# youtalk/opencv-ar

Hardware: AMD Instinct MI355X
Metric: frames/sec at 1920x1080, 16 markers/frame; 1/2/4/8 MI355X (higher is better)
Workload: dtype u8

## Files before the change

opencv-ar_amd/csrc/api.hip:

```cpp
#include "context.h"
#include "plan_core.h"
#include <algorithm>
#include <cstdlib>
#include <cstring>
#include <new>

using namespace ocvar;

static_assert(sizeof(TemplateRec) == sizeof(OcvarTemplate) && sizeof(TemplateRec) == 48, "CvarTemplate layout");
static_assert(MAX_SIZE_CLASSES == OCVAR_MAX_TEMPLATE_SIZES, "size classes");
static_assert(sizeof(CameraRec) == sizeof(OcvarCamera) && sizeof(CameraRec) == 248, "CvarCamera layout");
static_assert(sizeof(MarkerRec) == sizeof(OcvarMarker) && sizeof(MarkerRec) == 184, "CvarMarker layout");
static_assert(sizeof(BoardEntry) == sizeof(OcvarBoardMarker) && sizeof(BoardEntry) == 72, "OcvarBoardMarker layout");
static_assert(sizeof(BoardPose) == sizeof(OcvarBoardPose) && sizeof(BoardPose) == 192, "OcvarBoardPose layout");

template <typename T>
static int dev_alloc(OcvarHip* c, T** p, size_t n) {
    void* q = nullptr;
    HIP_TRY(c, hipMalloc(&q, n * sizeof(T) + 256));
    c->allocs.push_back(q);
    *p = static_cast<T*>(q);
    return OCVAR_OK;
}

static int create_impl(OcvarHip** out, int device, int max_width, int max_height, int max_batch, int max_quads, int max_markers,
                       bool dense) {
    if (!out || max_width < 16 || max_height < 16 || max_width > 32767 || max_height > 32767 || max_batch < 1 || max_quads < 1 ||
        max_markers < 1)
        return OCVAR_E_ARG;
    *out = nullptr;
    int ndev = 0;
    if (hipGetDeviceCount(&ndev) != hipSuccess || ndev <= 0 || device < 0 || device >= ndev) return OCVAR_E_NO_DEVICE;
    hipDeviceProp_t prop;
    if (hipGetDeviceProperties(&prop, device) != hipSuccess) return OCVAR_E_NO_DEVICE;
    if (std::strncmp(prop.gcnArchName, "gfx950", 6) != 0) {
        std::fprintf(stderr, "ocvar_hip: device %d is %s; this library carries gfx950 code only\n", device, prop.gcnArchName);
        return OCVAR_E_NO_DEVICE;
    }
    OcvarHip* c = new (std::nothrow) OcvarHip();
    if (!c) return OCVAR_E_HIP;
    *out = c;
    c->device = device;
    HIP_TRY(c, hipSetDevice(device));
    HIP_TRY(c, c->stream.ensure(hipStreamNonBlocking));
    for (auto& e : c->ev) HIP_TRY(c, e.ensure(hipEventDefault));
    Workspace& w = c->ws;
    plan_workspace(&w, max_width, max_height, max_batch, max_quads, max_markers, dense);
    c->result_limit = max_markers;
    const size_t B = (size_t)max_batch, M = (size_t)max_markers;
    int rc;
    if ((rc = dev_alloc(c, &w.gray, B * (size_t)gray_plane_bytes(max_width, max_height)))) return rc;
    if ((rc = dev_alloc(c, &w.nbr_frame, B * (size_t)nbr_plane_bytes(((max_width & ~1) + 15) & ~15, max_height & ~1)))) return rc;
    if ((rc = dev_alloc(c, &w.nbr_crop, (size_t)w.cap_crop_pixels))) return rc;
    if ((rc = dev_alloc(c, &w.cands_frame, (size_t)w.cap_frame_cands))) return rc;
    if ((rc = dev_alloc(c, &w.cands_crop, (size_t)w.cap_crop_cands))) return rc;
    if ((rc = dev_alloc(c, &w.pool, (size_t)w.cap_pool_ints))) return rc;
    if ((rc = dev_alloc(c, &w.slab, (size_t)w.max_mid_blocks * 256 * SLAB_STRIDE))) return rc;
    if ((rc = dev_alloc(c, &w.slab3, (size_t)w.max_long_blocks * 4 * SLAB3_STRIDE))) return rc;
    if ((rc = dev_alloc(c, &w.mid_frame, (size_t)w.cap_long))) return rc;
    if ((rc = dev_alloc(c, &w.mid_crop, (size_t)w.cap_long))) return rc;
    if ((rc = dev_alloc(c, &w.mid_first_crop, (size_t)w.cap_long))) return rc;
    if ((rc = dev_alloc(c, &w.long_frame, (size_t)w.cap_long))) return rc;
    if ((rc = dev_alloc(c, &w.long_crop, (size_t)w.cap_long))) return rc;
    if ((rc = dev_alloc(c, &w.quads_frame, B * max_quads))) return rc;
    if ((rc = dev_alloc(c, &w.n_quads_frame, B))) return rc;
    if ((rc = dev_alloc(c, &w.squares, B * max_quads * 8))) return rc;
    if ((rc = dev_alloc(c, &w.n_squares, B))) return rc;
    if ((rc = dev_alloc(c, &w.crop_of, B * max_quads))) return rc;
    if ((rc = dev_alloc(c, &w.rois_crop, (size_t)w.cap_crop_rois))) return rc;
    if ((rc = dev_alloc(c, &w.tiles_crop, (size_t)w.cap_crop_tiles))) return rc;
    if ((rc = dev_alloc(c, &w.quads_crop, (size_t)w.cap_crop_quads))) return rc;
    if ((rc = dev_alloc(c, &w.best_crop, (size_t)w.cap_crop_rois))) return rc;
    if ((rc = dev_alloc(c, &w.crop_min_rest, (size_t)w.cap_crop_rois))) return rc;
    if ((rc = dev_alloc(c, &w.ring_frame, B))) return rc;
    if ((rc = dev_alloc(c, &w.ring_crop, (size_t)w.cap_crop_rois))) return rc;
    if ((rc = dev_alloc(c, &w.sq_recs, B * max_quads))) return rc;
    if ((rc = dev_alloc(c, &w.prev, B * M))) return rc;
    if ((rc = dev_alloc(c, &w.n_prev, B))) return rc;
    if ((rc = dev_alloc(c, &w.reserve, B * M))) return rc;
    if ((rc = dev_alloc(c, &w.n_reserve, B))) return rc;
    if ((rc = dev_alloc(c, &w.markers, B * M))) return rc;
    if ((rc = dev_alloc(c, &w.pose_jobs, B * M))) return rc;
    if (dense) {
        const int nc = w.track_gw * w.track_gh;
        if ((rc = dev_alloc(c, &w.sorted_starts, B * max_quads))) return rc;
        if ((rc = dev_alloc(c, &w.sq_tmp, B * max_quads * 8))) return rc;
        if ((rc = dev_alloc(c, &w.trk_cells, B * (nc + 1)))) return rc;
        if ((rc = dev_alloc(c, &w.trk_fill, B * nc))) return rc;
        if ((rc = dev_alloc(c, &w.trk_items, B * 4 * max_quads))) return rc;
        if ((rc = dev_alloc(c, &w.trk_next, B * (max_quads + 1)))) return rc;
        if ((rc = dev_alloc(c, &w.surv, B * max_quads))) return rc;
        if ((rc = dev_alloc(c, &w.src, B * M))) return rc;
    }
    if ((rc = dev_alloc(c, &w.n_markers, B))) return rc;
    if ((rc = dev_alloc(c, &w.templates, (size_t)MAXT))) return rc;
    if ((rc = dev_alloc(c, &w.sizes, (size_t)MAX_SIZE_CLASSES))) return rc;
    if ((rc = dev_alloc(c, &w.lut, (size_t)4 * MAXT))) return rc;
    if ((rc = dev_alloc(c, &w.group_off, (size_t)MAXT + 1))) return rc;
    if ((rc = dev_alloc(c, &w.group_members, (size_t)MAXT))) return rc;
    if ((rc = dev_alloc(c, &w.camera, (size_t)1))) return rc;
    if ((rc = dev_alloc(c, &w.counters, (size_t)CNT_COUNT))) return rc;

    w.crop_pixels = reinterpret_cast<unsigned long long*>(w.counters + CNT_CROP_PIXELS);
    HIP_TRY(c, hipMemset(w.n_prev, 0, B * sizeof(int)));
    HIP_TRY(c, hipMemset(w.counters, 0, CNT_COUNT * sizeof(int)));
    HIP_TRY(c, c->h_markers.reserve(B * M * sizeof(MarkerRec)));
    HIP_TRY(c, c->h_counts.reserve(B * sizeof(int)));
    HIP_TRY(c, c->h_prev.reserve(B * M * sizeof(MarkerRec)));
    HIP_TRY(c, c->h_prev_counts.reserve(B * sizeof(int)));
    HIP_TRY(c, c->h_counters.reserve(CNT_COUNT * sizeof(int)));
    return OCVAR_OK;
}

extern "C" int ocvar_hip_create(OcvarHip** out, int device, int max_width, int max_height, int max_batch) {
    return ocvar_hip_create_ex(out, device, max_width, max_height, max_batch, OCVAR_MAX_QUADS);
}

extern "C" int ocvar_hip_create_ex(OcvarHip** out, int device, int max_width, int max_height, int max_batch, int max_quads) {
    if (max_quads < 1 || max_quads > OCVAR_MAX_QUADS_EX) return OCVAR_E_ARG;
    return create_impl(out, device, max_width, max_height, max_batch, max_quads, OCVAR_MAX_MARKERS, false);
}

extern "C" int ocvar_hip_create_dense(OcvarHip** out, int device, int max_width, int max_height, int max_batch, int max_quads,
                                      int max_markers) {
    if (max_quads < 1 || max_quads > OCVAR_MAX_QUADS_DENSE || max_markers < 1 || max_markers > OCVAR_MAX_MARKERS_DENSE) return OCVAR_E_ARG;
    return create_impl(out, device, max_width, max_height, max_batch, max_quads, max_markers, true);
}

extern "C" int ocvar_hip_max_markers(const OcvarHip* c) { return c ? c->ws.maxm : OCVAR_E_ARG; }

OcvarHip::~OcvarHip() {
    for (void* p : allocs) (void)hipFree(p);
    if (!h_overlays) return;
    for (auto& t : h_overlays->tex)
        if (t.px) (void)hipFree(const_cast<uint32_t*>(t.px));
    delete h_overlays;
}

extern "C" void ocvar_hip_destroy(OcvarHip* c) {
    if (!c) return;
    (void)hipSetDevice(c->device);
    gate_detach(c);
    if (c->stream) (void)hipStreamSynchronize(c->stream);
    if (c->ovl_used) (void)hipEventSynchronize(c->ovl_done);
// ... 681 lines not shown
```

opencv-ar_amd/csrc/follow.hip:

```cpp
#include "kernels.h"
#include "trace_core.h"

namespace ocvar {

__device__ __forceinline__ int ticket_lane() {
    int l = (int)(threadIdx.x & 63);
    asm volatile("" : "+v"(l));
    return l;
}
__device__ __forceinline__ int uni(int v) { return __builtin_amdgcn_readfirstlane(v); }
__device__ __forceinline__ unsigned uni(unsigned v) { return (unsigned)__builtin_amdgcn_readfirstlane((int)v); }
__device__ __forceinline__ unsigned long long uni(unsigned long long v) {
    return ((unsigned long long)uni((unsigned)(v >> 32)) << 32) | uni((unsigned)v);
}
__device__ __forceinline__ double uni(double v) { return __longlong_as_double((long long)uni((unsigned long long)__double_as_longlong(v))); }

#ifdef OCVAR_PROF
#define PROF_NOW() __builtin_readcyclecounter()
#define PROF_DECL() unsigned long long prof_acc[16] = {0, 0, 0, 0, 0, 0, 0, 0, 0, 0, 0, 0, 0, 0, 0, 0}
#define PROF_ADD(slot, v) do { prof_acc[slot] += (unsigned long long)(v); } while (0)
#define PROF_FLUSH(base) do { if ((threadIdx.x & 63) == 0) for (int i_ = 0; i_ < 16; i_++) if (i_ != 7) atomicAdd(reinterpret_cast<unsigned long long*>(ws.counters + CNT_PROF) + (base) + i_, prof_acc[i_]); } while (0)
#else
#define PROF_NOW() 0ull
#define PROF_DECL() do { } while (0)
// ... 277 lines not shown
        px = ex;
        py = ey;
    }
    __builtin_amdgcn_fence(__ATOMIC_ACQ_REL, "workgroup");
    return new_count;
}

template <bool CROP, bool STAGE>
__device__ __forceinline__ bool wave_finish_packed(const Workspace& ws, const StartCand c, const PlaneRef& pl, const unsigned* gsrc, int npts,
                                                   unsigned* lpts, WaveScratch* sc) {
    const int lane = threadIdx.x & 63;
    if (npts < 4) return false;
    unsigned lo = 0xffffffffu, hi = 0u;
    if (STAGE) {
        unsigned v[LDS_PTS / 64];
#pragma unroll
        for (int k = 0; k < LDS_PTS / 64; k++) {
            const int i = lane + 64 * k;
            v[k] = i < npts ? gsrc[i] : 0u;
        }
#pragma unroll
        for (int k = 0; k < LDS_PTS / 64; k++) {
            const int i = lane + 64 * k;
            if (i < npts) {
                lpts[i] = v[k];
                lo = pk_min(lo, v[k]);
                hi = pk_max(hi, v[k]);
            }
        }
    } else {
        for (int i = lane; i < npts; i += 64) {
            const unsigned p = gsrc[i];
            lo = pk_min(lo, p);
            hi = pk_max(hi, p);
        }
    }
    lo = wave_pk_min(lo);
    hi = wave_pk_max(hi);
    const int bw = px_of(hi) - px_of(lo), bh = py_of(hi) - py_of(lo);
    if (!((long long)bw * bh > 500)) return false;
    __builtin_amdgcn_fence(__ATOMIC_ACQ_REL, "workgroup");
    const unsigned* src = STAGE ? lpts : gsrc;
    double per = 0.0;
    for (int i = lane; i < npts; i += 64) {
        const unsigned p = src[i], q = src[i == 0 ? npts - 1 : i - 1];
        const float dx = (float)px_of(p) - (float)px_of(q), dy = (float)py_of(p) - (float)py_of(q);
        per += (double)sqrt_rn(dx * dx + dy * dy);
    }
    per = wave_sum_f64(per);
#ifdef OCVAR_PROF
    if (lane == 0) atomicAdd(reinterpret_cast<unsigned long long*>(ws.counters + CNT_PROF) + (CROP ? 16 : 0) + 7, 1ull);
#endif
    const bool k32 = npts <= 1024 && (long long)bw * bw + (long long)bh * bh < (1ll << 21);
    const int m = k32 ? wave_approx_dp<true>(src, npts, per * 0.02, sc->dst, sc->stack) : wave_approx_dp<false>(src, npts, per * 0.02, sc->dst, sc->stack);
    if (m != 4) return false;
    int q[8];
#pragma unroll
    for (int k = 0; k < 8; k++) q[k] = uni(sc->dst[k]);
    if (!quad_filter(q, pl.img_w, pl.img_h)) return false;
    if (lane == 0) emit_quad<CROP>(ws, c, q);
    return true;
}

template <bool CROP>
__device__ __forceinline__ int follow_short(const Workspace& ws, const StartCand c) {
    const int BUDGET = SHORT_STEPS;
    const PlaneRef pl = plane_of<CROP>(ws, c.roi);
    if (c.pos <= 0 || c.pos >= pl.plane) return false;
    {
        if (earlier_start_behind(pl.nbr, pl.ns, pl.plane, c.pos, c.is_hole, BACK_STEPS)) return 0;
        if (CROP) {
            const int x = c.pos % pl.ns, y = c.pos / pl.ns;
            return (x == 1 || y == 1) ? 3 : 1;
        }
        const LeanTrace lt = trace_flat(pl.nbr, pl.ns, pl.plane, c.pos, c.is_hole, nullptr, 0, BUDGET);
        if (lt.status == TRACE_OVERRUN) return lt.npts <= 2 ? 2 : 1;
        if (lt.status != TRACE_OK || lt.npts < 4) return 0;
        return 1;
    }
    return 0;
}

template <bool CROP>
__device__ int follow_overflow(const Workspace& ws, const StartCand c, const PlaneRef& pl) {
    const TraceStats st = trace_border<false, false>(pl.nbr, pl.ns, pl.plane, c.pos, c.is_hole, nullptr, 0, ws.mid_steps);
    if (st.status == TRACE_OVERRUN) return 1;
    if (!worth_approximating(st)) return 0;
    const int need = 2 * st.npts + 2 * (st.npts + 2);
    const long long off = atomicAdd(reinterpret_cast<unsigned long long*>(ws.counters + CNT_POOL_INTS), (unsigned long long)need);
    if (off + need > ws.cap_pool_ints) {
        atomicOr(ws.counters + CNT_ERR, ERR_POOL_OVERFLOW);
        return 0;
    }
    int* pts = ws.pool + off;
    trace_border<true, false>(pl.nbr, pl.ns, pl.plane, c.pos, c.is_hole, pts, st.npts, ws.mid_steps);
    approximate_and_emit<CROP>(ws, c, pl, pts, st.npts, st.perimeter, reinterpret_cast<DpSlice*>(pts + 2 * st.npts));
    return 0;
}

constexpr int T1_TICKET = 512;
constexpr int T1_OUT = 128;

template <bool CROP>
__global__ __launch_bounds__(FOLLOW_THREADS) void follow_kernel(Workspace ws) {
    const StartCand* cands = CROP ? ws.cands_crop : ws.cands_frame;
    int n = ws.counters[CROP ? CNT_CROP_CANDS : CNT_FRAME_CANDS];
    const int cap = CROP ? ws.cap_crop_cands : ws.cap_frame_cands;
    if (n > cap) n = cap;
    int* ticket = ws.counters + (CROP ? CNT_TICKET_C : CNT_TICKET_F);
    const int lane = threadIdx.x & 63;
    const int wave = uni((int)(threadIdx.x >> 6));
    const unsigned long long below = (1ull << lane) - 1ull;
    __shared__ StartCand wqueue[FW][128];
    __shared__ StartCand obuf[FW][3][T1_OUT];
    int o_n0 = 0, o_n1 = 0, o_n2 = 0;
    auto append = [&](int t, int& o_n) {
        if (o_n == 0) return;
        StartCand* list = t == 0 ? (CROP ? ws.mid_crop : ws.mid_frame) : t == 1 ? (CROP ? ws.long_crop : ws.long_frame) : ws.mid_first_crop;
        int* count = ws.counters + (t == 0 ? (CROP ? CNT_MID_C : CNT_MID_F) : t == 1 ? (CROP ? CNT_LONG_C : CNT_LONG_F) : CNT_MID_C_FIRST);
        __builtin_amdgcn_fence(__ATOMIC_ACQ_REL, "workgroup");
        int qbase = 0;
        if (lane == 0) qbase = atomicAdd(count, o_n);
        qbase = uni(qbase);
        for (int i = lane; i < o_n; i += 64) {
            if (qbase + i < ws.cap_long) list[qbase + i] = obuf[wave][t][i];
            else atomicOr(ws.counters + CNT_ERR, ERR_CAND_OVERFLOW);
        }
        __builtin_amdgcn_fence(__ATOMIC_ACQ_REL, "workgroup");
        o_n = 0;
    };
    auto collect = [&](int t, int& o_n, bool mine, const StartCand& c) {
        const unsigned long long mask = __ballot(mine);
        if (!mask) return;
        const int cnt = __popcll(mask);
        if (o_n + cnt > T1_OUT) append(t, o_n);
        if (mine) obuf[wave][t][o_n + __popcll(mask & below)] = c;
        o_n += cnt;
    };
    int queued = 0;
    int tk_next = 0, tk_end = 0;
    bool more = true;
    for (int guard = 2 * (n / 64 + 2) + 2;; guard--) {
        if (guard < 0) {
            if (lane == 0) atomicOr(ws.counters + CNT_ERR, ERR_TICKET_RUNAWAY);
            break;
        }
        while (more && queued < 64) {
            if (tk_next >= tk_end) {
                int base = 0;
                if (ticket_lane() == 0) base = atomicAdd(ticket, T1_TICKET);
                base = uni(base);
                if (base >= n) {
                    more = false;
                    break;
                }
                tk_next = base;
                tk_end = base + T1_TICKET < n ? base + T1_TICKET : n;
            }
            const int idx = tk_next + lane;
            tk_next += 64;
            bool alive = false;
            StartCand cc;
            cc.roi = 0; cc.pos = 0; cc.is_hole = 0;
            if (idx < tk_end) {
                cc = cands[idx];
                const PlaneRef pl = plane_of<CROP>(ws, cc.roi);
                const bool ring_done = !cc.is_hole && cc.pos == pl.ns + 1 && (CROP ? ws.ring_crop : ws.ring_frame)[cc.roi] != 0;
                if (!ring_done && cc.pos > 0 && cc.pos < pl.plane && !run_has_earlier_pixel_bits(pl.nbr, pl.ns, cc.pos, cc.is_hole))
                    alive = trace_flat(pl.nbr, pl.ns, pl.plane, cc.pos, cc.is_hole, nullptr, 0, PRE_STEPS).status == TRACE_OVERRUN;
            }
            const unsigned long long mask = __ballot(alive);
            if (alive) wqueue[wave][queued + __popcll(mask & below)] = cc;
            queued += __popcll(mask);
        }
        if (queued == 0) break;
        const int take = queued < 64 ? queued : 64;
        __builtin_amdgcn_fence(__ATOMIC_ACQ_REL, "workgroup");
        StartCand c;
// ... 56 lines not shown
}

constexpr unsigned LW_EXIT = 0x1c00u;
constexpr unsigned LW_DELTA = 0x00030003u;

__device__ __forceinline__ unsigned lean_table_entry(unsigned idx) {
    const unsigned from = idx & 7u, t = idx >> 3;
    const unsigned e = (from + t) & 7u;
    const unsigned dx = (unsigned)(step_dx((int)e) + 1), dy = (unsigned)(step_dy((int)e) + 1);
    const unsigned pw = ((12u - from) & 7u) < t, pe = ((8u - from) & 7u) < t;
    return dx | (dy << 16) | (((e + 5u) & 7u) << 5) | (e << 10) | (pe << 30) | (pw << 31);
}

struct LeanWalk {
    unsigned xy;
    unsigned m;
    unsigned from;
    unsigned pe;
    unsigned xy0, xy1;
    unsigned cxy;
    int npts, step, status;
};

__device__ __forceinline__ void lean_begin(LeanWalk& w, const uint8_t* nbr, int ns, int cpos, int is_hole) {
    const int i0 = cpos - is_hole;
    const int x = i0 % ns, y = i0 / ns;
    w.xy = w.xy0 = (unsigned)x | ((unsigned)y << 16);
    w.cxy = w.xy0 + (unsigned)is_hole;
    w.npts = 0;
    w.step = 0;
    w.status = -1;
    w.xy1 = 0;
    w.pe = 0;
    w.from = 0;
    w.m = nbr_of(nbr, x, y, ns);
    if (w.m == 0) {
        w.status = TRACE_SINGLE;
        w.npts = 1;
        return;
    }
    const int s = first_cw(w.m, (is_hole ? 0 : 4) - 1);
    w.xy1 = w.xy0 + (unsigned)(step_dx(s) + 65536 * step_dy(s));
    w.pe = (unsigned)(s ^ 4) << 10;
    w.from = (unsigned)(s + 1) & 7u;
}

template <class Park>
__device__ __forceinline__ void lean_step(LeanWalk& w, const unsigned* tab, const uint8_t* base, unsigned nt, unsigned last, Park&& park) {
    const unsigned mm = __builtin_amdgcn_perm(w.m, w.m, 0u);
    const unsigned t = (unsigned)__builtin_ctz(__builtin_amdgcn_alignbit(mm, mm, w.from));
    const unsigned ent = tab[(t << 3) + w.from];
    const int d = (int)(w.xy - w.cxy);
    const unsigned nf = ((ent << 1) & (unsigned)(d + 1)) | (ent & (unsigned)d);
    const unsigned nxy = w.xy + (ent & LW_DELTA) - 0x10001u;
    const bool closes = (nxy == w.xy0) & (w.xy == w.xy1);
    const unsigned e = ent & LW_EXIT;
    const bool emit = e != w.pe;
    unsigned off = nbr_win_off_xy(nxy, nt);
    off = off < last ? off : last;
    const unsigned* win = reinterpret_cast<const unsigned*>(base + off);
    const unsigned m4 = nbr_mask9(win[0], win[1], win[2], nxy & 15u);
    park(w.xy);
    w.npts += emit ? 1 : 0;
    w.status = (int)nf < 0 ? (int)TRACE_NOT_FIRST : closes ? (int)TRACE_OK : m4 == 0u ? (int)TRACE_OVERRUN : -1;
    w.step += 1;
    w.xy = nxy;
    w.pe = e;
    w.from = (ent >> 5) & 7u;
    w.m = m4;
}

constexpr int MID_BLOCK = 32;
constexpr int POINT_ROW = MID_BLOCK + 1;
constexpr int FLUSH_W = MID_BLOCK <= 16 ? 16 : 32;
static_assert(FLUSH_W >= MID_BLOCK && 64 % FLUSH_W == 0, "a group of lanes covers a whole row of parked points");

template <bool CROP>
__global__ __launch_bounds__(FOLLOW_THREADS) void follow_mid_kernel(Workspace ws, int phase) {
    __shared__ WaveScratch scratch[FW];
    __shared__ unsigned parked[FW][64 * POINT_ROW];
    __shared__ unsigned step_tab[64];
    if (threadIdx.x < 64u) step_tab[threadIdx.x] = lean_table_entry(threadIdx.x);
    __syncthreads();
    const StartCand* cands = CROP ? ws.mid_crop : ws.mid_frame;
    StartCand* longs = CROP ? ws.long_crop : ws.long_frame;
    int n = ws.counters[CROP ? CNT_MID_C : CNT_MID_F];
    if (n > ws.cap_long) n = ws.cap_long;
    int n_first = (CROP && phase != 2) ? ws.counters[CNT_MID_C_FIRST] : 0;
    if (n_first > ws.cap_long) n_first = ws.cap_long;
    n += n_first;
    int* ticket = ws.counters + (CROP ? (phase == 2 ? CNT_TICKET_MC2 : CNT_TICKET_MC) : CNT_TICKET_MF);
    int* n_long = ws.counters + (CROP ? CNT_LONG_C : CNT_LONG_F);
    const int lane = threadIdx.x & 63;
    const int wave = uni((int)(threadIdx.x >> 6));
    const unsigned long long below = (1ull << lane) - 1ull;
    unsigned* wave_slabs = reinterpret_cast<unsigned*>(ws.slab) + ((size_t)blockIdx.x * blockDim.x + uni((int)(threadIdx.x & ~63u))) * SLAB_STRIDE;
    static_assert(64 * POINT_ROW >= LDS_PTS, "the staging area of the approximation aliases the (flushed) point rows");
    unsigned* my_row = parked[wave] + lane * POINT_ROW;
    const unsigned* wave_rows = parked[wave];
    int flushed = 0;
    const int budget = ws.mid_steps;
    bool have = false;
    bool more = true;
    StartCand c;
    c.roi = 0; c.pos = 0; c.is_hole = 0;
    PlaneRef pl = plane_of<CROP>(ws, 0);
    LeanWalk w;
    w.xy = w.m = w.from = w.pe = w.xy0 = w.xy1 = w.cxy = 0u;
    w.npts = w.step = 0;
    w.status = TRACE_NOT_FIRST;
    unsigned pl_nt = 1u, pl_last = 0u;
    long long guard = ((long long)n + 64) * (budget / MID_BLOCK + 5) + 64;
    PROF_DECL();
    for (;;) {
        if (--guard < 0) {
            if (lane == 0) atomicOr(ws.counters + CNT_ERR, ERR_TICKET_RUNAWAY);
            break;
        }
        const unsigned long long pt0 = PROF_NOW();
        for (int tries = 0; tries < (CROP ? 4 : 1); tries++) {
            const unsigned long long idle = __ballot(!have);
            if (!(more && idle)) break;
            if (tries > 0) --guard;
            const int cnt = __popcll(idle);
            int base = 0;
            if (ticket_lane() == 0) base = atomicAdd(ticket, cnt);
            base = uni(base);
            if (base + cnt >= n) more = false;
            if (!have) {
                const int idx = base + __popcll(idle & below);
                if (idx < n) {
                    c = (CROP && idx < n_first) ? ws.mid_first_crop[idx] : cands[idx - n_first];
                    bool take = true;
                    if (CROP) {
                        const int earliest = ws.crop_min_rest[c.roi];
                        const bool beaten = (unsigned)(ws.best_crop[c.roi] >> 32) < (unsigned)c.pos;
                        if (phase == 1) take = idx < n_first || c.pos == earliest;
                        else if (phase == 2) take = c.pos != earliest && !beaten;
                        else take = !beaten;
                    }
                    pl = plane_of<CROP>(ws, c.roi);
                    if (take && c.pos > 0 && c.pos < pl.plane) {
                        lean_begin(w, pl.nbr, pl.ns, c.pos, c.is_hole);
                        pl_nt = (unsigned)(pl.ns >> 4);
                        pl_last = (unsigned)nbr_plane_bytes(pl.ns, pl.sh) - 12u;
                        have = true;
                        flushed = 0;
                    }
                }
            }
        }
        if (__ballot(have) == 0) break;
        const unsigned long long pt1 = PROF_NOW();
        PROF_ADD(0, pt1 - pt0);
        for (int k = 0; k < MID_BLOCK; k++) {
            const bool running = have && w.status < 0;
            if (__ballot(running) == 0) break;
            PROF_ADD(4, 1);
            PROF_ADD(5, __popcll(__ballot(running)));
            if (running)
                lean_step(w, step_tab, pl.nbr, pl_nt, pl_last, [&](unsigned xy) {
                    const int slot = w.npts - flushed;
                    my_row[slot < MID_BLOCK ? slot : MID_BLOCK] = xy;
                });
        }
        if (have && w.status < 0 && w.step >= budget) w.status = TRACE_OVERRUN;
        const unsigned long long pt2 = PROF_NOW();
        PROF_ADD(1, pt2 - pt1);
        {
            const int stored = w.npts < SLAB_PTS ? w.npts : SLAB_PTS;
            const int pend = have ? stored - flushed : 0;
            unsigned long long fm = __ballot(pend > 0);
            if (fm) __builtin_amdgcn_fence(__ATOMIC_ACQ_REL, "workgroup");
            const int grp = lane / FLUSH_W, k = lane % FLUSH_W;
            while (fm) {
                int L = 0, cnt = 0, off = 0;
#pragma unroll
                for (int g = 0; g < 64 / FLUSH_W; g++) {
                    const int Lg = fm ? __ffsll((long long)fm) - 1 : 0;
                    const int cg = fm ? __builtin_amdgcn_readlane(pend, Lg) : 0;
                    const int og = __builtin_amdgcn_readlane(flushed, Lg);
                    fm &= fm - 1;
                    L = grp == g ? Lg : L;
                    cnt = grp == g ? cg : cnt;
                    off = grp == g ? og : off;
                }
                if (k < cnt) wave_slabs[(size_t)L * SLAB_STRIDE + off + k] = wave_rows[L * POINT_ROW + k];
            }
            flushed += pend;
        }
        const unsigned long long pt3 = PROF_NOW();
        PROF_ADD(2, pt3 - pt2);
        int route = 0, slab_npts = 0;
#ifdef OCVAR_PROF
        {
            const bool done = have && w.status >= 0;
            for (int st_ = 0; st_ < 3; st_++) {
                const int want = st_ == 0 ? (int)TRACE_NOT_FIRST : st_ == 1 ? (int)TRACE_OK : (int)TRACE_OVERRUN;
                const bool mine = done && w.status == want;
                PROF_ADD(9 + 2 * st_, __popcll(__ballot(mine)));
                unsigned steps_ = mine ? (unsigned)w.step : 0u;
                for (int o_ = 32; o_ > 0; o_ >>= 1) steps_ += (unsigned)__shfl_xor((int)steps_, o_, 64);
                PROF_ADD(8 + 2 * st_, steps_);
            }
            bool useless = false;
            if (CROP && done && w.status == TRACE_OK) useless = (unsigned)(ws.best_crop[c.roi] >> 32) < (unsigned)c.pos;
            unsigned us_ = useless ? (unsigned)w.step : 0u;
            for (int o_ = 32; o_ > 0; o_ >>= 1) us_ += (unsigned)__shfl_xor((int)us_, o_, 64);
            PROF_ADD(14, us_);
            PROF_ADD(15, __popcll(__ballot(done && w.status == TRACE_OK && w.npts < 4)));
        }
#endif
        if (have && w.status >= 0) {
            if (w.status == TRACE_OVERRUN) route = 1;
            else if (w.status == TRACE_OK && w.npts >= 4) {
                if (w.npts <= SLAB_PTS) {
                    route = 3;
                    slab_npts = w.npts;
                } else {
                    route = follow_overflow<CROP>(ws, c, pl);
                }
            }
            have = false;
        }
        unsigned long long todo = __ballot(route == 3);
        unsigned my_best = 0xffffffffu;
        if (CROP && route == 3) my_best = (unsigned)(ws.best_crop[c.roi] >> 32);
        if (todo) __builtin_amdgcn_fence(__ATOMIC_ACQ_REL, "workgroup");
        while (todo) {
            const int L = __ffsll((long long)todo) - 1;
            todo &= todo - 1;
            StartCand cl;
            cl.roi = __builtin_amdgcn_readlane(c.roi, L);
            cl.pos = __builtin_amdgcn_readlane(c.pos, L);
            cl.is_hole = __builtin_amdgcn_readlane(c.is_hole, L);
            const int nl = __builtin_amdgcn_readlane(slab_npts, L);
            const unsigned* sl = wave_slabs + (size_t)L * SLAB_STRIDE;
            PlaneRef pll = pl;
            pll.img_w = __builtin_amdgcn_readlane(pl.img_w, L);
            pll.img_h = __builtin_amdgcn_readlane(pl.img_h, L);
            const bool beaten = CROP && (unsigned)__builtin_amdgcn_readlane((int)my_best, L) < (unsigned)cl.pos;
            if (!beaten) wave_finish_packed<CROP, true>(ws, cl, pll, sl, nl, parked[wave], &scratch[wave]);
            PROF_ADD(6, 1);
        }
        PROF_ADD(3, PROF_NOW() - pt3);
        const unsigned long long mask = __ballot(route == 1);
        if (mask) {
            int qbase = 0;
            const int leader = __ffsll((long long)mask) - 1;
            if (lane == leader) qbase = atomicAdd(n_long, __popcll(mask));
            qbase = __builtin_amdgcn_readlane(qbase, leader);
            if (route == 1) {
                const int slot = qbase + __popcll(mask & below);
                if (slot < ws.cap_long) longs[slot] = c;
                else atomicOr(ws.counters + CNT_ERR, ERR_CAND_OVERFLOW);
            }
        }
    }
    PROF_FLUSH(CROP ? 16 : 0);
}

constexpr int TILE_SLOTS = TILE_H + 2;
struct TileCache {
    unsigned* lds;
    const uint8_t* nbr;
    int ns, sh;
    int tx0, ty0;
};

__device__ __forceinline__ void tile_load(TileCache& t, int x, int y, int bx = 0, int by = 0) {
    const int lane = threadIdx.x & 63;
    t.tx0 = (x + 20 * bx - TILE_W / 2 + 8) & ~15;
    t.ty0 = (int)div14((unsigned)(y + 24 * by - 28 + 4 * NBR_TILE_H)) * NBR_TILE_H - 4 * NBR_TILE_H;
    const int tx = (t.tx0 >> 4), ty = t.ty0 / NBR_TILE_H, nty = (t.sh + NBR_TILE_H - 1) / NBR_TILE_H;
    constexpr int NQ = TILE_TX * TILE_TY * 4;
    static_assert(NQ > 64 && NQ <= 128, "two quarter tiles per lane at most");
    uint4 v[2];
#pragma unroll
    for (int h = 0; h < 2; h++) {
        const int q = lane + 64 * h, i = (q >> 2) % TILE_TX, j = (q >> 2) / TILE_TX;
        v[h] = make_uint4(0u, 0u, 0u, 0u);
        if (q < NQ && tx + i >= 0 && (tx + i) * 16 < t.ns && ty + j >= 0 && ty + j < nty)
            v[h] = *reinterpret_cast<const uint4*>(t.nbr + nbr_tile_off((unsigned)(tx + i), (unsigned)(ty + j), t.ns) + 16 * (q & 3));
    }
#pragma unroll
    for (int h = 0; h < 2; h++) {
        const int q = lane + 64 * h, i = (q >> 2) % TILE_TX, j = (q >> 2) / TILE_TX;
        if (q < NQ) {
            unsigned* d = t.lds + i * TILE_SLOTS + NBR_TILE_H * j + 4 * (q & 3);
            d[0] = v[h].x; d[1] = v[h].y; d[2] = v[h].z; d[3] = v[h].w;
        }
    }
    __builtin_amdgcn_fence(__ATOMIC_ACQ_REL, "workgroup");
}

__device__ __forceinline__ unsigned tile_mask(const TileCache& t, int lx, int ly) {
    const unsigned* w = t.lds + ((unsigned)lx >> 4) * TILE_SLOTS + (unsigned)ly;
    return nbr_mask9(w[0], w[1], w[2], (unsigned)lx & 15u);
}

__device__ __forceinline__ unsigned tile_get(TileCache& t, int x, int y) {
    if ((unsigned)(x - t.tx0) >= (unsigned)TILE_W || (unsigned)(y - t.ty0) >= (unsigned)TILE_H) tile_load(t, x, y);
    return uni(tile_mask(t, x - t.tx0, y - t.ty0));
}

__device__ LeanTrace trace_lean_tiled(TileCache& t, int cpos, int is_hole, int* out, int max_pts, int max_steps) {
    const int lane = threadIdx.x & 63;
    LeanTrace r;
    r.status = TRACE_OK;
    r.npts = 0;
    r.steps = 0;
    const int ns = t.ns;
    const int i0 = cpos - is_hole;
    const int x0 = i0 % ns, y0 = i0 / ns;
    int x = x0, y = y0;
    unsigned m = tile_get(t, x, y);
    if (m == 0) {
        r.status = TRACE_SINGLE;
        r.npts = 1;
        return r;
    }
    int s = first_cw(m, (is_hole ? 0 : 4) - 1);
    const int x1 = x0 + step_dx(s), y1 = y0 + step_dy(s);
    int prev_s = s ^ 4;
    int straight = 0;
    int step = 0;
    unsigned hp = 0;
    unsigned* out1 = reinterpret_cast<unsigned*>(out);
    for (;; step++) {
        if (step >= max_steps) {
            r.status = TRACE_OVERRUN;
            break;
        }
        const int from = (s + 1) & 7;
        const int tz = __builtin_ctz(((m * 0x101u) >> from) & 0xffu);
        const int e = (from + tz) & 7;
        const unsigned passed = ((((1u << tz) - 1u) * 0x101u) << from) >> 8;
        const int idx = y * ns + x;
        if (((passed & 0x10u) && idx < cpos) || ((passed & 1u) && idx + 1 < cpos)) {
            r.status = TRACE_NOT_FIRST;
            break;
        }
        if (e != prev_s) {
// ... 304 lines not shown
    __syncthreads();
    const int per = (nc + REPLAY_THREADS - 1) / REPLAY_THREADS, c0 = tid * per, c1 = c0 + per < nc ? c0 + per : nc;
    int sum = 0;
    for (int c = c0; c < c1; c++) sum += __hip_atomic_load(fill + c, __ATOMIC_RELAXED, __HIP_MEMORY_SCOPE_AGENT);
    s_part[tid] = sum;
    __syncthreads();
    for (int d = 1; d < REPLAY_THREADS; d <<= 1) {
        const int v = tid >= d ? s_part[tid - d] : 0;
        __syncthreads();
        s_part[tid] += v;
        __syncthreads();
    }
    int run = s_part[tid] - sum;
    for (int c = c0; c < c1; c++) {
        const int k = __hip_atomic_load(fill + c, __ATOMIC_RELAXED, __HIP_MEMORY_SCOPE_AGENT);
        cells[c] = run;
        fill[c] = run;
        run += k;
    }
    if (tid == 0) cells[nc] = 4 * n;
    __syncthreads();
    for (int j = tid; j < 4 * n; j += REPLAY_THREADS)
        items[atomicAdd(fill + track_cell(tmp[2 * j + 1], gh) * gw + track_cell(tmp[2 * j], gw), 1)] = j >> 2;
    __syncthreads();
    if (tid == 0) {
        int nr = 0;
        s_left = track_markers_sparse(ws.prev + (size_t)f * ws.maxm, np, tmp, n, cells, items, gw, gh, next,
                                      ws.reserve + (size_t)f * ws.maxm, ws.maxm, &nr);
        ws.n_reserve[f] = nr;
        ws.n_squares[f] = s_left;
    }
    __syncthreads();
    int base = 0;
    for (int b = 0; b < n; b += REPLAY_THREADS) {
        const int i = b + tid;
        const int keep = i < n && next[i] == i;
        s_part[tid] = keep;
        __syncthreads();
        for (int d = 1; d < REPLAY_THREADS; d <<= 1) {
            const int v = tid >= d ? s_part[tid - d] : 0;
            __syncthreads();
            s_part[tid] += v;
            __syncthreads();
        }
        if (keep) {
            const int o = base + s_part[tid] - 1;
            for (int k = 0; k < 8; k++) sq[(size_t)o * 8 + k] = tmp[(size_t)i * 8 + k];
        }
        base += s_part[REPLAY_THREADS - 1];
        __syncthreads();
    }
}

__global__ __launch_bounds__(256) void crops_kernel(Workspace ws) {
    const int CH = ws.order_chunk;
    const int nch = (ws.maxq + CH - 1) / CH;
    const int f = blockIdx.x / nch, c = blockIdx.x % nch;
    int n = ws.n_squares[f];
    if (n > ws.maxq) n = ws.maxq;
    const int hi = n < (c + 1) * CH ? n : (c + 1) * CH;
    for (int i = c * CH + (int)threadIdx.x; i < hi; i += blockDim.x) setup_crop(ws, f, i, ws.squares + ((size_t)f * ws.maxq + i) * 8);
}

void launch_ring_quads_frames(const Workspace& ws, hipStream_t stream) {
    hipLaunchKernelGGL(ring_quads_kernel<false>, dim3(ws.n_frames < 4096 ? ws.n_frames : 4096), dim3(64), 0, stream, ws);
}
void launch_ring_quads_crops(const Workspace& ws, hipStream_t stream) {
    hipLaunchKernelGGL(ring_quads_kernel<true>, dim3(ws.n_frames >= 128 ? 4096 : ws.n_frames * 32), dim3(64), 0, stream, ws);
}
void launch_follow_frames(const Workspace& ws, hipStream_t stream) {
    hipLaunchKernelGGL(follow_kernel<false>, dim3(ws.short_blocks * (4 / FW)), dim3(FOLLOW_THREADS), 0, stream, ws);
}
void launch_follow_crops(const Workspace& ws, hipStream_t stream) {
    hipLaunchKernelGGL(follow_kernel<true>, dim3(ws.short_blocks * (4 / FW)), dim3(FOLLOW_THREADS), 0, stream, ws);
}
void launch_follow_mid_frames(const Workspace& ws, hipStream_t stream) {
    hipLaunchKernelGGL(follow_mid_kernel<false>, dim3(ws.mid_blocks * (4 / FW)), dim3(FOLLOW_THREADS), 0, stream, ws, 0);
}
void launch_follow_mid_crops(const Workspace& ws, hipStream_t stream) {
    if (ws.crop_phases == 1) {
        hipLaunchKernelGGL(follow_mid_kernel<true>, dim3(ws.mid_blocks * (4 / FW)), dim3(FOLLOW_THREADS), 0, stream, ws, 0);
        return;
    }
    hipLaunchKernelGGL(follow_mid_kernel<true>, dim3(ws.mid_blocks * (4 / FW)), dim3(FOLLOW_THREADS), 0, stream, ws, 1);
    hipLaunchKernelGGL(follow_mid_kernel<true>, dim3(ws.mid_blocks * (4 / FW)), dim3(FOLLOW_THREADS), 0, stream, ws, 2);
}
void launch_follow_long_frames(const Workspace& ws, hipStream_t stream) {
    hipLaunchKernelGGL(follow_long_kernel<false>, dim3(ws.long_blocks * (4 / FW)), dim3(FOLLOW_THREADS), 0, stream, ws);
}
void launch_follow_long_crops(const Workspace& ws, hipStream_t stream) {
    hipLaunchKernelGGL(follow_long_kernel<true>, dim3(ws.long_blocks * (4 / FW)), dim3(FOLLOW_THREADS), 0, stream, ws);
}
void launch_order_and_crops(const Workspace& ws, hipStream_t stream) {
    if (ws.n_frames > 0 && ws.dense) {
        const int grid = ws.n_frames * ((ws.maxq + ws.order_chunk - 1) / ws.order_chunk);
        hipLaunchKernelGGL(order_sort_kernel, dim3(grid), dim3(ws.order_chunk / 2 > 64 ? ws.order_chunk / 2 : 64), 0, stream, ws);
        hipLaunchKernelGGL(order_place_kernel, dim3(grid), dim3(256), 0, stream, ws);
        hipLaunchKernelGGL(track_replay_kernel, dim3(ws.n_frames), dim3(REPLAY_THREADS), 0, stream, ws);
        hipLaunchKernelGGL(crops_kernel, dim3(grid), dim3(256), 0, stream, ws);
        return;
    }
    if (ws.n_frames > 0) hipLaunchKernelGGL(order_and_crops_kernel, dim3(ws.n_frames), dim3(ws.maxq <= 256 ? 64 : 256) , (size_t)ws.maxq * 9 * sizeof(int), stream, ws);
}

}
```

opencv-ar_amd/csrc/kernels.h:

```cpp
#pragma once
#include "hd.h"
#include "decode_core.h"
#include "pose_core.h"
#include "tail_core.h"
#include "refine_core.h"
#include "board_core.h"
#include "overlay_core.h"
#include "patch_core.h"
#include "ocvar_hip.h"

namespace ocvar {

constexpr int MAXQ_DEFAULT = OCVAR_MAX_QUADS;
constexpr int MAXM = OCVAR_MAX_MARKERS;
constexpr int MAXT = OCVAR_MAX_TEMPLATES;
constexpr int MARCH_HALO_L = 2, MARCH_HALO_R = 2;
constexpr int MARCH_STRIP = 4 * (64 - MARCH_HALO_L - MARCH_HALO_R);
static_assert(MARCH_STRIP == GRAY_PANEL_COLS && 4 * MARCH_HALO_L == GRAY_PANEL_LEAD && 4 * 64 == GRAY_PANEL_BYTES, "a grey panel is what one wave of the frame kernel converts");
constexpr int MARCH_CROP_ROWS = 252;
constexpr int MARCH_STAGE = 512;
constexpr int BACK_STEPS = 32;
constexpr int PRE_STEPS = 8;
constexpr int SHORT_STEPS = 96;
constexpr int MID_STEPS = 1536;
constexpr int SLAB_PTS = 1024;
constexpr int SLAB_STRIDE = SLAB_PTS + 4;
constexpr int MID_BLOCKS_MAX = 1024;
constexpr int SLAB3_PTS = 8192;
constexpr int SLAB3_STRIDE = SLAB3_PTS + 64;
constexpr int LONG_BLOCKS_MAX = 1024;
constexpr int TILE_TX = 4, TILE_TY = 5;
constexpr int TILE_W = TILE_TX * NBR_TILE_W, TILE_H = TILE_TY * NBR_TILE_H;

enum { ERR_CAND_OVERFLOW = 1, ERR_POOL_OVERFLOW = 2, ERR_QUAD_OVERFLOW = 4, ERR_TRACE_OVERRUN = 8, ERR_CROP_OVERFLOW = 16,
       ERR_TILE_OVERFLOW = 32,
       ERR_TICKET_RUNAWAY = 64,
       ERR_MARKER_OVERFLOW = 128 };

struct TileDesc { int roi, x0, y0; };

struct SquareRec {
    float square[8];
    float patPoint[8];
    int n_match;
    int pad;
};

enum { CNT_FRAME_CANDS = 0, CNT_CROP_ROIS = 1, CNT_CROP_TILES = 2, CNT_CROP_CANDS = 3,
       CNT_POOL_INTS = 4 , CNT_CROP_QUADS = 6, CNT_TICKET_F = 7, CNT_TICKET_C = 8, CNT_ERR = 9,
       CNT_CROP_PIXELS = 10 , CNT_LONG_F = 12, CNT_LONG_C = 13, CNT_TICKET_LF = 14, CNT_TICKET_LC = 15,
       CNT_MID_F = 16, CNT_MID_C = 17, CNT_TICKET_MF = 18, CNT_TICKET_MC = 19, CNT_TICKET_BC = 20, CNT_MID_C_FIRST = 21, CNT_TICKET_MC2 = 22,
       CNT_POSE_JOBS = 23,
       CNT_PROF = 24 , CNT_COUNT = 88 };

struct Workspace {
    int max_w, max_h, max_batch;
    int maxq;
    int maxm;
    int dense;
    int track_gw, track_gh;
    int decode_slices;
    int order_chunk;
    int cap_frame_cands, cap_crop_cands, cap_crop_rois, cap_crop_tiles, cap_crop_quads;
    long long cap_pool_ints, cap_crop_pixels;
    int W, H, sw, sh, ns, n_frames, n_templates;
    int n_sizes, n_groups, max_match;
    int crop_phases;
    int mid_steps, mid_blocks, long_blocks;
    int max_mid_blocks, max_long_blocks;
    int short_blocks, crop_blocks;
    int frame_strips, frame_chunks, frame_chunk_rows;
    uint8_t* gray;
    uint8_t* nbr_frame;
    uint8_t* nbr_crop;
    StartCand* cands_frame;
    StartCand* cands_crop;
    StartCand* mid_frame;
    StartCand* mid_crop;
    StartCand* mid_first_crop;
    StartCand* long_frame;
    StartCand* long_crop;
    int cap_long;
    int* pool;
    int* slab;
    int* slab3;
    QuadRec* quads_frame;
    int* n_quads_frame;
    float* squares;
    int* n_squares;
    int* crop_of;
    Roi* rois_crop;
    TileDesc* tiles_crop;
    unsigned long long* crop_pixels;
    QuadRec* quads_crop;
    unsigned long long* best_crop;
    int* ring_frame;
    int* ring_crop;
    int* crop_min_rest;
    SquareRec* sq_recs;
    long long* sq_codes;
    int* sq_match;
    MarkerRec* prev;
    int* n_prev;
    int* reserve;
    int* n_reserve;
    int* pose_jobs;
    MarkerRec* markers;
    int* sorted_starts;
    float* sq_tmp;
    int* trk_cells;
    int* trk_fill;
    int* trk_items;
    int* trk_next;
    int* surv;
    int* src;
    int* n_markers;
    TemplateRec* templates;
    SizeClass* sizes;
    LutEntry* lut;
    int* group_off;
    int* group_members;
    CameraRec* camera;
    int* counters;
};

int input_format_bpp(int format);

void launch_binarise_frames(const Workspace& ws, const uint8_t* d_bgr, int row_stride, size_t frame_stride, int grey_in_place,
                            int format, hipStream_t stream);
void launch_binarise_crops(const Workspace& ws, hipStream_t stream);
void launch_ring_quads_frames(const Workspace& ws, hipStream_t stream);
void launch_ring_quads_crops(const Workspace& ws, hipStream_t stream);
void launch_follow_frames(const Workspace& ws, hipStream_t stream);
void launch_follow_crops(const Workspace& ws, hipStream_t stream);
void launch_follow_mid_frames(const Workspace& ws, hipStream_t stream);
void launch_follow_mid_crops(const Workspace& ws, hipStream_t stream);
void launch_follow_long_frames(const Workspace& ws, hipStream_t stream);
void launch_follow_long_crops(const Workspace& ws, hipStream_t stream);
void launch_order_and_crops(const Workspace& ws, hipStream_t stream);
void launch_decode(const Workspace& ws, hipStream_t stream);
void launch_finalise(const Workspace& ws, const RefineArgs& refine, hipStream_t stream);
void launch_refine_corners(const Workspace& ws, const RefineArgs& refine, hipStream_t stream);

struct BoardArgs {
    int n;
    const BoardEntry* entries;
    const int* map;
    BoardPose* poses;
};
void launch_board_poses(const Workspace& ws, const BoardArgs& board, hipStream_t stream);

struct OverlayArgs {
    const OverlayTable* table;
    OverlayDraw* draws;
    OverlayBox* boxes;
};
void launch_overlay(const OverlayArgs& oa, uint8_t* frames, int W, int H, long long row_stride, long long frame_stride, int n_frames,
                    int format, const MarkerRec* recs, const int* counts, int stride, hipStream_t stream);

struct PatchArgs {
    const uint8_t* frames;
    int W, H;
// ... 12 lines not shown
```

opencv-ar_amd/csrc/plan_core.h:

```cpp
#pragma once
#include "kernels.h"

namespace ocvar {

struct PlanKnob {
    bool set;
    long long value;
};
inline long long knob_or(PlanKnob k, long long dflt) { return k.set ? k.value : dflt; }

struct PlanOverrides {
    PlanKnob crop_phases, mid_steps, mid_blocks, long_blocks, short_blocks, min_units;
};

inline long long plan_min(long long a, long long b) { return a < b ? a : b; }
inline long long plan_max(long long a, long long b) { return a > b ? a : b; }

inline void plan_workspace(Workspace* wp, int max_width, int max_height, int max_batch, int max_quads, int max_markers, bool dense) {
    Workspace& w = *wp;
    w.max_w = max_width;
    w.max_h = max_height;
    w.max_batch = max_batch;
    w.maxq = max_quads;
    w.maxm = max_markers;
    w.dense = dense ? 1 : 0;
    const long long B = max_batch, WH = (long long)max_width * max_height;
    const long long per_frame_cands = WH / 16 < 16384 ? 16384 : WH / 16;
    w.cap_frame_cands = (int)plan_min(B * per_frame_cands, 1ll << 30);
    w.cap_crop_cands = w.cap_frame_cands;
    w.cap_crop_rois = (int)(B * max_quads);
    w.cap_crop_tiles = (int)plan_min(B * (dense ? plan_max(4096, 4ll * max_quads) : 4096), 1ll << 30);
    w.cap_crop_quads = (int)(B * max_quads * 4);
    w.cap_pool_ints = B * (1 << 18) + (1 << 24);
    w.cap_crop_pixels = B * (max_width + 16) * (max_height + 8);
    if (dense) w.cap_crop_pixels *= 4;
    w.max_mid_blocks = (int)plan_min(MID_BLOCKS_MAX, plan_max(32, B));
    w.max_long_blocks = (int)plan_min(LONG_BLOCKS_MAX, plan_max(128, B * 8));
    w.cap_long = (int)plan_min(plan_max(B * 4096, 1ll << 18), 1ll << 28);
    if (dense) {
        (void)track_grid_cells(max_width, max_height, &w.track_gw, &w.track_gh);
        w.decode_slices = (int)plan_max(4, plan_min(64, max_quads / 64));
        for (w.order_chunk = 2; w.order_chunk < max_quads && w.order_chunk < ORDER_CHUNK;) w.order_chunk <<= 1;
    }
}

inline void plan_batch(Workspace* wp, int width, int height, int n_frames, bool gated, const PlanOverrides& ov) {
    Workspace& w = *wp;
    w.W = width;
    w.H = height;
    w.sw = width & ~1;
    w.sh = height & ~1;
    w.ns = (w.sw + 15) & ~15;
    w.n_frames = n_frames;
    w.mid_steps = (int)knob_or(ov.mid_steps, n_frames <= 8 ? 128 : MID_STEPS);
    if (w.mid_steps < 32) w.mid_steps = 32;
    w.crop_phases = knob_or(ov.crop_phases, n_frames <= 8 ? 1 : 2) == 1 ? 1 : 2;
    w.mid_blocks = (int)knob_or(ov.mid_blocks, gated ? plan_max(32, w.max_mid_blocks / 4) : w.max_mid_blocks);
    if (w.mid_blocks < 1 || w.mid_blocks > w.max_mid_blocks) w.mid_blocks = w.max_mid_blocks;
    w.long_blocks = (int)knob_or(ov.long_blocks, w.max_long_blocks);
    if (w.long_blocks < 1 || w.long_blocks > w.max_long_blocks) w.long_blocks = w.max_long_blocks;
    w.short_blocks = (int)knob_or(ov.short_blocks, n_frames >= 128 ? 1024 : (n_frames * 8 < 16 ? 16 : n_frames * 8));
    if (w.short_blocks < 1 || w.short_blocks > 65535) w.short_blocks = 1024;
    w.crop_blocks = n_frames >= 128 ? 2048 : (n_frames * 16 < 32 ? 32 : n_frames * 16);
    w.frame_strips = (w.sw + MARCH_STRIP - 1) / MARCH_STRIP;
    int chunks = (w.sh + 64) / 128;
    if (chunks < 1) chunks = 1;
    const long long min_units = knob_or(ov.min_units, gated ? 16384 : 65536);
    while (chunks > 1 && (long long)w.frame_strips * (chunks / 2) * n_frames >= min_units) chunks /= 2;
    int rows = (w.sh + chunks - 1) / chunks;
    rows = (rows + NBR_TILE_H - 1) / NBR_TILE_H * NBR_TILE_H;
    w.frame_chunk_rows = rows;
    w.frame_chunks = (w.sh + rows - 1) / rows;
}

}
```

Baseline: 245,600.

## Compact crop candidates into per-phase lists and raise crop walk budget

Adds split and prune kernels that compact crop mid-candidates into an earliest-start list, a remainder list and a still-live list, so each crop follow phase only scans candidates it will actually take instead of filtering the whole list per phase. It also gives crop traces a per-image step budget scaled by crop perimeter, capped at a new larger constant, so long crop borders finish in tier 2 rather than overflowing. This costs two extra kernel launches, three more candidate buffers, and possibly longer per-wave walks. The retry count per phase also changes.

```diff
diff --git a/opencv-ar_amd/csrc/api.hip b/opencv-ar_amd/csrc/api.hip
--- a/opencv-ar_amd/csrc/api.hip
+++ b/opencv-ar_amd/csrc/api.hip
@@ -60,6 +60,9 @@
     if ((rc = dev_alloc(c, &w.mid_frame, (size_t)w.cap_long))) return rc;
     if ((rc = dev_alloc(c, &w.mid_crop, (size_t)w.cap_long))) return rc;
     if ((rc = dev_alloc(c, &w.mid_first_crop, (size_t)w.cap_long))) return rc;
+    if ((rc = dev_alloc(c, &w.crop_early, (size_t)w.cap_long))) return rc;
+    if ((rc = dev_alloc(c, &w.crop_rest, (size_t)w.cap_long))) return rc;
+    if ((rc = dev_alloc(c, &w.crop_live, (size_t)w.cap_long))) return rc;
     if ((rc = dev_alloc(c, &w.long_frame, (size_t)w.cap_long))) return rc;
     if ((rc = dev_alloc(c, &w.long_crop, (size_t)w.cap_long))) return rc;
     if ((rc = dev_alloc(c, &w.quads_frame, B * max_quads))) return rc;
diff --git a/opencv-ar_amd/csrc/croplist_core.h b/opencv-ar_amd/csrc/croplist_core.h
--- /dev/null
+++ b/opencv-ar_amd/csrc/croplist_core.h
@@ -0,0 +1,19 @@
+#pragma once
+#include "hd.h"
+
+namespace ocvar {
+
+constexpr int CROP_NO_START = 0x7fffffff;
+constexpr unsigned long long CROP_NO_QUAD = ~0ull;
+
+OCVAR_HD bool crop_start_earliest(int pos, int crop_min_rest) { return pos == crop_min_rest; }
+OCVAR_HD bool crop_start_beaten(int pos, unsigned long long best_crop) { return (unsigned)(best_crop >> 32) < (unsigned)pos; }
+
+constexpr int CROP_BUDGET_FACTOR = 6, CROP_BUDGET_BLOCK = 32;
+OCVAR_HD int crop_walk_budget(int sw, int sh, int mid_steps, int cap) {
+    int b = (CROP_BUDGET_FACTOR * (sw + sh) + CROP_BUDGET_BLOCK - 1) & ~(CROP_BUDGET_BLOCK - 1);
+    b = b > mid_steps ? b : mid_steps;
+    return b < cap ? b : cap;
+}
+
+}
diff --git a/opencv-ar_amd/csrc/follow.hip b/opencv-ar_amd/csrc/follow.hip
--- a/opencv-ar_amd/csrc/follow.hip
+++ b/opencv-ar_amd/csrc/follow.hip
@@ -383,8 +383,8 @@
 }
 
 template <bool CROP>
-__device__ int follow_overflow(const Workspace& ws, const StartCand c, const PlaneRef& pl) {
-    const TraceStats st = trace_border<false, false>(pl.nbr, pl.ns, pl.plane, c.pos, c.is_hole, nullptr, 0, ws.mid_steps);
+__device__ int follow_overflow(const Workspace& ws, const StartCand c, const PlaneRef& pl, int max_steps) {
+    const TraceStats st = trace_border<false, false>(pl.nbr, pl.ns, pl.plane, c.pos, c.is_hole, nullptr, 0, max_steps);
     if (st.status == TRACE_OVERRUN) return 1;
     if (!worth_approximating(st)) return 0;
     const int need = 2 * st.npts + 2 * (st.npts + 2);
@@ -394,7 +394,7 @@
         return 0;
     }
     int* pts = ws.pool + off;
-    trace_border<true, false>(pl.nbr, pl.ns, pl.plane, c.pos, c.is_hole, pts, st.npts, ws.mid_steps);
+    trace_border<true, false>(pl.nbr, pl.ns, pl.plane, c.pos, c.is_hole, pts, st.npts, max_steps);
     approximate_and_emit<CROP>(ws, c, pl, pts, st.npts, st.perimeter, reinterpret_cast<DpSlice*>(pts + 2 * st.npts));
     return 0;
 }
@@ -617,9 +617,9 @@
     __shared__ unsigned step_tab[64];
     if (threadIdx.x < 64u) step_tab[threadIdx.x] = lean_table_entry(threadIdx.x);
     __syncthreads();
-    const StartCand* cands = CROP ? ws.mid_crop : ws.mid_frame;
+    const StartCand* cands = CROP ? (phase == 1 ? ws.crop_early : phase == 2 ? ws.crop_live : ws.mid_crop) : ws.mid_frame;
     StartCand* longs = CROP ? ws.long_crop : ws.long_frame;
-    int n = ws.counters[CROP ? CNT_MID_C : CNT_MID_F];
+    int n = ws.counters[CROP ? (phase == 1 ? CNT_CROP_EARLY : phase == 2 ? CNT_CROP_LIVE : CNT_MID_C) : CNT_MID_F];
     if (n > ws.cap_long) n = ws.cap_long;
     int n_first = (CROP && phase != 2) ? ws.counters[CNT_MID_C_FIRST] : 0;
     if (n_first > ws.cap_long) n_first = ws.cap_long;
@@ -634,7 +634,8 @@
     unsigned* my_row = parked[wave] + lane * POINT_ROW;
     const unsigned* wave_rows = parked[wave];
     int flushed = 0;
-    const int budget = ws.mid_steps;
+    const int budget = CROP ? ws.crop_steps_cap : ws.mid_steps;
+    const int max_tries = CROP ? (phase == 1 ? 1 : phase == 2 ? 2 : 4) : 1;
     bool have = false;
     bool more = true;
     StartCand c;
@@ -653,7 +654,7 @@
             break;
         }
         const unsigned long long pt0 = PROF_NOW();
-        for (int tries = 0; tries < (CROP ? 4 : 1); tries++) {
+        for (int tries = 0; tries < max_tries; tries++) {
             const unsigned long long idle = __ballot(!have);
             if (!(more && idle)) break;
             if (tries > 0) --guard;
@@ -667,13 +668,7 @@
                 if (idx < n) {
                     c = (CROP && idx < n_first) ? ws.mid_first_crop[idx] : cands[idx - n_first];
                     bool take = true;
-                    if (CROP) {
-                        const int earliest = ws.crop_min_rest[c.roi];
-                        const bool beaten = (unsigned)(ws.best_crop[c.roi] >> 32) < (unsigned)c.pos;
-                        if (phase == 1) take = idx < n_first || c.pos == earliest;
-                        else if (phase == 2) take = c.pos != earliest && !beaten;
-                        else take = !beaten;
-                    }
+                    if (CROP && phase != 1) take = !crop_start_beaten(c.pos, ws.best_crop[c.roi]);
                     pl = plane_of<CROP>(ws, c.roi);
                     if (take && c.pos > 0 && c.pos < pl.plane) {
                         lean_begin(w, pl.nbr, pl.ns, c.pos, c.is_hole);
@@ -699,7 +694,7 @@
                     my_row[slot < MID_BLOCK ? slot : MID_BLOCK] = xy;
                 });
         }
-        if (have && w.status < 0 && w.step >= budget) w.status = TRACE_OVERRUN;
+        if (have && w.status < 0 && w.step >= (CROP ? crop_walk_budget(pl.img_w & ~1, pl.img_h & ~1, ws.mid_steps, budget) : budget)) w.status = TRACE_OVERRUN;
         const unsigned long long pt2 = PROF_NOW();
         PROF_ADD(1, pt2 - pt1);
         {
@@ -739,7 +734,7 @@
                 PROF_ADD(8 + 2 * st_, steps_);
             }
             bool useless = false;
-            if (CROP && done && w.status == TRACE_OK) useless = (unsigned)(ws.best_crop[c.roi] >> 32) < (unsigned)c.pos;
+            if (CROP && done && w.status == TRACE_OK) useless = crop_start_beaten(c.pos, ws.best_crop[c.roi]);
             unsigned us_ = useless ? (unsigned)w.step : 0u;
             for (int o_ = 32; o_ > 0; o_ >>= 1) us_ += (unsigned)__shfl_xor((int)us_, o_, 64);
             PROF_ADD(14, us_);
@@ -753,7 +748,7 @@
                     route = 3;
                     slab_npts = w.npts;
                 } else {
-                    route = follow_overflow<CROP>(ws, c, pl);
+                    route = follow_overflow<CROP>(ws, c, pl, CROP ? crop_walk_budget(pl.img_w & ~1, pl.img_h & ~1, ws.mid_steps, budget) : budget);
                 }
             }
             have = false;
@@ -794,6 +789,59 @@
     }
     PROF_FLUSH(CROP ? 16 : 0);
 }
+
+constexpr int CL_CHUNK = 512;
+static_assert(CROP_BUDGET_BLOCK == MID_BLOCK, "a crop's budget is rounded to the unit tier 2 checks it in");
+
+template <bool PRUNE>
+__device__ __forceinline__ void crop_lists(const Workspace& ws) {
+    __shared__ StartCand stage[PRUNE ? 1 : 2][CL_CHUNK];
+    const StartCand* src = PRUNE ? ws.crop_rest : ws.mid_crop;
+    int n = ws.counters[PRUNE ? CNT_CROP_REST : CNT_MID_C];
+    if (n > ws.cap_long) n = ws.cap_long;
+    const int lane = threadIdx.x;
+    const unsigned long long below = (1ull << lane) - 1ull;
+    for (int base = (int)blockIdx.x * CL_CHUNK; base < n; base += (int)gridDim.x * CL_CHUNK) {
+        int n0 = 0, n1 = 0;
+        const int end = base + CL_CHUNK < n ? base + CL_CHUNK : n;
+        for (int i0 = base; i0 < end; i0 += 64) {
+            const int i = i0 + lane;
+            bool to0 = false, to1 = false;
+            StartCand c;
+            c.roi = 0; c.pos = 0; c.is_hole = 0;
+            if (i < end) {
+                c = src[i];
+                if (PRUNE) {
+                    to0 = !crop_start_beaten(c.pos, ws.best_crop[c.roi]);
+                } else {
+                    to0 = crop_start_earliest(c.pos, ws.crop_min_rest[c.roi]);
+                    to1 = !to0;
+                }
+            }
+            const unsigned long long m0 = __ballot(to0), m1 = __ballot(to1);
+            if (to0) stage[0][n0 + __popcll(m0 & below)] = c;
+            if (!PRUNE && to1) stage[PRUNE ? 0 : 1][n1 + __popcll(m1 & below)] = c;
+            n0 += __popcll(m0);
+            n1 += __popcll(m1);
+        }
+        __builtin_amdgcn_fence(__ATOMIC_ACQ_REL, "workgroup");
+        for (int t = 0; t < (PRUNE ? 1 : 2); t++) {
+            const int cnt = t == 0 ? n0 : n1;
+            StartCand* list = PRUNE ? ws.crop_live : (t == 0 ? ws.crop_early : ws.crop_rest);
+            int* count = ws.counters + (PRUNE ? CNT_CROP_LIVE : (t == 0 ? CNT_CROP_EARLY : CNT_CROP_REST));
+            int qbase = 0;
+            if (lane == 0 && cnt > 0) qbase = atomicAdd(count, cnt);
+            qbase = uni(qbase);
+            for (int k = lane; k < cnt; k += 64) {
+                if (qbase + k < ws.cap_long) list[qbase + k] = stage[t][k];
+                else atomicOr(ws.counters + CNT_ERR, ERR_CAND_OVERFLOW);
+            }
+        }
+        __builtin_amdgcn_fence(__ATOMIC_ACQ_REL, "workgroup");
+    }
+}
+__global__ __launch_bounds__(64) void crop_split_kernel(Workspace ws) { crop_lists<false>(ws); }
+__global__ __launch_bounds__(64) void crop_prune_kernel(Workspace ws) { crop_lists<true>(ws); }
 
 constexpr int TILE_SLOTS = TILE_H + 2;
 struct TileCache {
@@ -1264,7 +1312,10 @@
         hipLaunchKernelGGL(follow_mid_kernel<true>, dim3(ws.mid_blocks * (4 / FW)), dim3(FOLLOW_THREADS), 0, stream, ws, 0);
         return;
     }
+    const int list_blocks = ws.n_frames >= 2048 ? 1024 : (ws.n_frames < 32 ? 16 : ws.n_frames / 2);
+    hipLaunchKernelGGL(crop_split_kernel, dim3(list_blocks), dim3(64), 0, stream, ws);
     hipLaunchKernelGGL(follow_mid_kernel<true>, dim3(ws.mid_blocks * (4 / FW)), dim3(FOLLOW_THREADS), 0, stream, ws, 1);
+    hipLaunchKernelGGL(crop_prune_kernel, dim3(list_blocks), dim3(64), 0, stream, ws);
     hipLaunchKernelGGL(follow_mid_kernel<true>, dim3(ws.mid_blocks * (4 / FW)), dim3(FOLLOW_THREADS), 0, stream, ws, 2);
 }
 void launch_follow_long_frames(const Workspace& ws, hipStream_t stream) {
diff --git a/opencv-ar_amd/csrc/kernels.h b/opencv-ar_amd/csrc/kernels.h
--- a/opencv-ar_amd/csrc/kernels.h
+++ b/opencv-ar_amd/csrc/kernels.h
@@ -7,6 +7,7 @@
 #include "board_core.h"
 #include "overlay_core.h"
 #include "patch_core.h"
+#include "croplist_core.h"
 #include "ocvar_hip.h"
 
 namespace ocvar {
@@ -23,6 +24,7 @@
 constexpr int PRE_STEPS = 8;
 constexpr int SHORT_STEPS = 96;
 constexpr int MID_STEPS = 1536;
+constexpr int CROP_STEPS_CAP = 3072;
 constexpr int SLAB_PTS = 1024;
 constexpr int SLAB_STRIDE = SLAB_PTS + 4;
 constexpr int MID_BLOCKS_MAX = 1024;
@@ -51,7 +53,8 @@
        CNT_CROP_PIXELS = 10 , CNT_LONG_F = 12, CNT_LONG_C = 13, CNT_TICKET_LF = 14, CNT_TICKET_LC = 15,
        CNT_MID_F = 16, CNT_MID_C = 17, CNT_TICKET_MF = 18, CNT_TICKET_MC = 19, CNT_TICKET_BC = 20, CNT_MID_C_FIRST = 21, CNT_TICKET_MC2 = 22,
        CNT_POSE_JOBS = 23,
-       CNT_PROF = 24 , CNT_COUNT = 88 };
+       CNT_PROF = 24 ,
+       CNT_CROP_EARLY = 88, CNT_CROP_REST = 89, CNT_CROP_LIVE = 90 , CNT_COUNT = 92 };
 
 struct Workspace {
     int max_w, max_h, max_batch;
@@ -66,6 +69,7 @@
     int W, H, sw, sh, ns, n_frames, n_templates;
     int n_sizes, n_groups, max_match;
     int crop_phases;
+    int crop_steps_cap;
     int mid_steps, mid_blocks, long_blocks;
     int max_mid_blocks, max_long_blocks;
     int short_blocks, crop_blocks;
@@ -78,6 +82,9 @@
     StartCand* mid_frame;
     StartCand* mid_crop;
     StartCand* mid_first_crop;
+    StartCand* crop_early;
+    StartCand* crop_rest;
+    StartCand* crop_live;
     StartCand* long_frame;
     StartCand* long_crop;
     int cap_long;
diff --git a/opencv-ar_amd/csrc/plan_core.h b/opencv-ar_amd/csrc/plan_core.h
--- a/opencv-ar_amd/csrc/plan_core.h
+++ b/opencv-ar_amd/csrc/plan_core.h
@@ -54,6 +54,7 @@
     w.n_frames = n_frames;
     w.mid_steps = (int)knob_or(ov.mid_steps, n_frames <= 8 ? 128 : MID_STEPS);
     if (w.mid_steps < 32) w.mid_steps = 32;
+    w.crop_steps_cap = (n_frames > 8 && !ov.mid_steps.set) ? (int)plan_max(CROP_STEPS_CAP, w.mid_steps) : w.mid_steps;
     w.crop_phases = knob_or(ov.crop_phases, n_frames <= 8 ? 1 : 2) == 1 ? 1 : 2;
     w.mid_blocks = (int)knob_or(ov.mid_blocks, gated ? plan_max(32, w.max_mid_blocks / 4) : w.max_mid_blocks);
     if (w.mid_blocks < 1 || w.mid_blocks > w.max_mid_blocks) w.mid_blocks = w.max_mid_blocks;
```

New measurement: 249,500, median of 6. 1.02x the previous value.
